# seshnadathur/victor

Measured on AMD Instinct MI355X. Metric: likelihood evals/sec (40 s-bins, 100 mu, l=0,2,4), higher is better.
Workload: dtype f64

## Files before the change

### victor_amd/csrc/vk_common.h

```cpp
#pragma once
#include <hip/hip_runtime.h>

#include "victor_hip.h"
#include "vk_devmath.h"
#include "vk_views.h"

namespace vk {

__device__ __forceinline__ int late_tid() {
  int t = threadIdx.x;
  asm volatile("" : "+v"(t));
  return t;
}


constexpr int kBlock = 256;
constexpr int kWaves = kBlock / 64;
constexpr int kMaxEll = 3;
constexpr int kVrVars = 5;
constexpr int kMaxParts = 8;


constexpr int kLikeRed = 4 * kWaves;
struct LikeArgs {
  const double* params;
  const double* theory;
  long long n;
  int N;
  int n_beta_d;
  const double* beta_d;
  const double* data;
  int n_beta_c;
  const double* beta_c;
  const double* prec;
  int grids_in_lds;
  const double* tri;
  const double* logdet;
  const double* eig;
  int like_form;
  double nmocks, nparams;
  double* lnl;
  double* chi2;
#ifdef VK_PHASES
  long long* stamps;
#endif
};

struct TheoryArgs {
  const double* params;
  long long n;
  int n_s, n_mu, n_x, n_ell;
  const double* s;
  const double* mu;
  const double* w_ell;
  const double* x;
  const double* w_x;
  const double* xw_scaled;
  double xw_max;
  const double* xgw;
  int n_xg;
  int n_beta_r;
  const double* beta_r;
  PPView xi, vr, sv;
  double iaH;
  double inv_sigma8;
  int rescale_from_ap;
  int matter_vt;
  double vt_amp;
  int sv_n_mu;
  double sv_mu_inv_h;
  const double* sv_mu;
  const double* sv2d;
  const double* sva;
  int sva_doubles;
  int uni_n;
  double uni_u0, uni_inv_h;
  const double* uni_sv_v;
  const double* uni_xi;
  const double* uni_xic;
  const double* uni_vb;
  const double* uni_v2;
  const double* uni_da;
  const double* uni_ge;
  const double* uni_dab;
  const double* uni_empb;
  int uni_lut_n;
  double uni_lut_inv_g;
  const unsigned short* uni_lut;
  const double* uni_knots;
  int matter_lb;
  int vr_beta_dep;
  const double* vr_emp;
  int from_data;
  int empirical;
  int rsd;
  int niter;
  int kaiser_approx;
  int coord_shift;
  int lanes_per_block;
  int sbins_per_item;
  int team;
  double* out;
  const double* exp_tab;
  const double* exp_tab_rep;
  const double* stage_mu;
  const double* image;
  double wsum[3];
  unsigned nx_magic;
  unsigned nmu_magic;
  unsigned ns_magic;
  int xi_out;
  int parts;
  int cells_per_item;
  int fuse;
  unsigned* counters;
  double* partial;
  int poll;
  int* poll_failed;
  LikeArgs like;
  double row0[VK_NPAR];
  int inline_row;
  int want_theory;
#ifdef VK_PHASES
  long long* stamps;
#endif
};

#ifdef VK_PHASES
#define VK_STAMP(a, k) do { if ((a).stamps && threadIdx.x == 0 && blockIdx.x < 4096) (a).stamps[blockIdx.x * 16 + (k)] = wall_clock64(); } while (0)
#else
#define VK_STAMP(a, k) do { } while (0)
#endif

struct PPLds {
  const double* knots;
  const double* coef;
  int n_int;
  int lead;
  double inv_h;
  double lo, hi, x_u0;
};

__device__ __forceinline__ int pp_interval(const PPLds& t, double u) {
  int i;
  if (t.inv_h != 0.0) {
    const int n_uniform = t.n_int - t.lead;
    const double tt = (u - t.x_u0) * fabs(t.inv_h);
    i = (int)tt;
    i = min(max(i, 0), n_uniform - 1) + t.lead;
    if (t.lead && u < t.x_u0) i = 0;
    if (t.inv_h < 0.0) {
      if (u < t.knots[i]) {
        i = max(i - 1, 0);
      } else if (u >= t.knots[i + 1]) {
        i = min(i + 1, t.n_int - 1);
      }
    }
  } else {
    int lo = 0, hi = t.n_int;
    while (hi - lo > 1) {
      int mid = (lo + hi) >> 1;
      if (u >= t.knots[mid]) lo = mid; else hi = mid;
    }
    i = lo;
  }
  return i;
}

__device__ __forceinline__ double pp_eval_at(const PPLds& t, int var, int i, double u) {
  const double dx = u - t.knots[i];
  const double* c = t.coef + ((size_t)var * t.n_int + i) * 4;
  return fma(fma(fma(c[3], dx, c[2]), dx, c[1]), dx, c[0]);
}

__device__ __forceinline__ double clampd(double u, double lo, double hi) { return fmin(fmax(u, lo), hi); }

__device__ __forceinline__ double wave_sum(double v) { return vkm::wave_sum(v); }

struct VelocityNode { double x, w; int last; };
__device__ __forceinline__ VelocityNode load_node(const double* xgw, int k) {
  typedef int node_words __attribute__((ext_vector_type(4)));
  typedef const node_words __attribute__((address_space(4))) * node_ptr;
  const node_words q = ((node_ptr)(unsigned long long)xgw)[k];
  VelocityNode n;
  n.x = __hiloint2double(q.y, q.x);
  n.w = __hiloint2double(q.w, q.z);
  n.last = q.w;
  return n;
}

template <int BYTES>
__device__ __forceinline__ void warm_kernarg_lines() {
  static_assert(BYTES <= 896, "extend the list of lines");
  const auto kp = __builtin_amdgcn_kernarg_segment_ptr();
  unsigned d0, d1, d2, d3, d4, d5, d6, d7, d8, d9, d10, d11;
  asm volatile(
      "s_load_dword %0, %12, 0x0\n\t"
      "s_load_dword %1, %12, 0x40\n\t"
      "s_load_dword %2, %12, 0x80\n\t"
      "s_load_dword %3, %12, 0xc0\n\t"
      "s_load_dword %4, %12, 0x100\n\t"
      "s_load_dword %5, %12, 0x140\n\t"
      "s_load_dword %6, %12, 0x180\n\t"
      "s_load_dword %7, %12, 0x1c0\n\t"
      "s_load_dword %8, %12, 0x200\n\t"
      "s_load_dword %9, %12, 0x240\n\t"
      "s_load_dword %10, %12, 0x280\n\t"
      "s_load_dword %11, %12, 0x2c0\n\t"
      "s_waitcnt lgkmcnt(0)"
      : "=&s"(d0), "=&s"(d1), "=&s"(d2), "=&s"(d3), "=&s"(d4), "=&s"(d5), "=&s"(d6), "=&s"(d7), "=&s"(d8), "=&s"(d9),
        "=&s"(d10), "=&s"(d11)
      : "s"(kp)
      : "memory");
  if constexpr (BYTES > 768) {
    unsigned e0, e1;
    if constexpr (BYTES > 832)
      asm volatile("s_load_dword %0, %2, 0x300\n\ts_load_dword %1, %2, 0x340\n\ts_waitcnt lgkmcnt(0)" : "=&s"(e0), "=&s"(e1) : "s"(kp) : "memory");
    else
      asm volatile("s_load_dword %0, %1, 0x300\n\ts_waitcnt lgkmcnt(0)" : "=&s"(e0) : "s"(kp) : "memory");
  }
}

__device__ __forceinline__ void store_shared(double* p, double v) {
  __hip_atomic_store(p, v, __ATOMIC_RELAXED, __HIP_MEMORY_SCOPE_AGENT);
}
__device__ __forceinline__ double load_shared(const double* p) {
  return __hip_atomic_load(p, __ATOMIC_RELAXED, __HIP_MEMORY_SCOPE_AGENT);
}

typedef double vk_shared2 __attribute__((ext_vector_type(2)));
__device__ __forceinline__ void load_shared_x8(const double* p, double (&v)[8]) {
  vk_shared2 a, b, c, d;
  asm volatile(
      "global_load_dwordx4 %0, %4, off sc1\n\t"
      "global_load_dwordx4 %1, %4, off offset:16 sc1\n\t"
      "global_load_dwordx4 %2, %4, off offset:32 sc1\n\t"
      "global_load_dwordx4 %3, %4, off offset:48 sc1\n\t"
      "s_waitcnt vmcnt(0)"
      : "=&v"(a), "=&v"(b), "=&v"(c), "=&v"(d)
      : "v"(p)
      : "memory");
  v[0] = a.x; v[1] = a.y; v[2] = b.x; v[3] = b.y; v[4] = c.x; v[5] = c.y; v[6] = d.x; v[7] = d.y;
}

constexpr unsigned long long kPollEmpty = 0x7ff8a5a57ff8a5a5ULL;
constexpr long long kPollTicks = 500000000LL;
__device__ __forceinline__ bool poll_is_empty(double v) { return (unsigned long long)__double_as_longlong(v) == kPollEmpty; }

__device__ __forceinline__ void drain_shared_stores() { asm volatile("s_waitcnt vmcnt(0)" ::: "memory"); }

__device__ __forceinline__ const double* param_row(const TheoryArgs& a, long long point) {
  return a.inline_row ? a.row0 : a.params + point * VK_NPAR;
}

__device__ __forceinline__ bool point_completed(unsigned* counters, long long point, unsigned total, int* flag) {
  drain_shared_stores();
  __syncthreads();
  if (threadIdx.x == 0) {
    const unsigned done = __hip_atomic_fetch_add(counters + point, 1u, __ATOMIC_RELAXED, __HIP_MEMORY_SCOPE_AGENT) + 1u;
    if (done == total) __hip_atomic_store(counters + point, 0u, __ATOMIC_RELAXED, __HIP_MEMORY_SCOPE_AGENT);
    *flag = done == total ? 1 : 0;
  }
  __syncthreads();
  return *flag != 0;
}

__device__ __forceinline__ double growth_amplitude(const TheoryArgs& a, const double* row, double fs8, double* av,
                                                   double* extra) {
  double growth = fs8 * a.inv_sigma8;
  double binv = 1.0;
  if (a.matter_lb) {
    const double bias = row[VK_P_BIAS];
    if (a.from_data) growth = row[VK_P_BETA] * bias;
    binv = vkm::recip(bias);
    *extra += bias;
  }
  if (a.matter_vt) growth = -3.0 * a.iaH * a.vt_amp * fs8;
  *av = 0.0;
  if (a.empirical && !a.matter_vt) {
    *av = row[VK_P_AV] * binv;
    *extra += *av;
  }
  return growth * binv;
}

struct PointScalars {
  double aperp, apar, inv_c, A, B;
  double G;
  double gD;
  double M, Q;
  double av;
  double inv_aperp, inv_apar;
  double poison;
};



__device__ __forceinline__ PointScalars point_scalars(const TheoryArgs& a, const double* row) {
  PointScalars ps;
  const double fs8 = row[VK_P_FSIGMA8];
  const double sigv = row[VK_P_SIGMAV];
  ps.aperp = row[VK_P_APERP];
  ps.apar = row[VK_P_APAR];
  const double eps = row[VK_P_EPSILON];
  double c;
  if (a.rescale_from_ap) {
    const int lane = threadIdx.x & 63;
    const double e2 = eps * eps - 1.0;
    const double h = (1.0 - 1e-10) / 49.0;
    double v = 0.0;
    if (lane < 50) {
      const double m = (lane == 49) ? 1.0 : fma((double)lane, h, 1e-10);
      double g, ir;
      vkm::sqrt_rsqrt(fma(1.0 - m * m, e2, 1.0), g, ir);
      v = ps.apar * g;
      if (lane == 0 || lane == 49) v *= 0.5;
    }
    c = wave_sum(v) * h;
  } else {
    c = row[VK_P_ASTAR];
  }
  ps.inv_c = vkm::recip(c);
  const double iaH_true = a.iaH * ps.apar;
  double extra = 0.0;
  const double gb = growth_amplitude(a, row, fs8, &ps.av, &extra);
  ps.B = sigv * iaH_true;
  ps.A = gb * vkm::recip(3.0 * iaH_true * sigv);
  ps.G = gb * (1.0 / 3.0);
  ps.gD = gb * ps.inv_c;
  ps.M = row[VK_P_M];
  ps.Q = row[VK_P_Q];
  ps.inv_aperp = vkm::recip(ps.aperp);
  ps.inv_apar = vkm::recip(ps.apar);
  ps.poison = 0.0 * (gb + sigv + ps.aperp + ps.apar + eps + c + ps.A + extra + (a.n_beta_r > 0 ? row[VK_P_BETA] : 0.0));
  return ps;
}

}
```

### victor_amd/csrc/vk_kernel_cells.h

```cpp
#pragma once
#include "vk_kernel_fast.h"

namespace vk {

struct CellsPlan {
  int mu, w, s, betar, da, v1, sva, image_end, acc, like, total;
};

__host__ __device__ inline int cells_range_bins(int n_mu, int cpi) { return (cpi + n_mu - 2) / n_mu + 1; }

__host__ __device__ inline CellsPlan make_cells_plan(int n_mu, int n_x, int n_s, int uni_n, int nlr, int n_beta_r,
                                                     int lut_n, int with_da, int cpi, int n_like, int n_sva = 0) {
  CellsPlan p;
  int o = fast_fixed_doubles(uni_n, nlr, lut_n);
  o = (o + 1) & ~1;
  p.mu = o;    o += 2 * n_mu;
  p.w = o;     o += kMaxEll * n_mu;
  p.s = o;     o += (n_s + 1) & ~1;
  p.betar = o; o += (n_beta_r + 1) & ~1;
  p.da = o;    o += with_da ? uni_n * 4 : 0;
  p.v1 = o;    o += with_da == 1 ? 0 : uni_n * 4;
  o = (o + 1) & ~1;
  p.sva = o;   o += (n_sva + 1) & ~1;
  p.image_end = o;
  int bins = cells_range_bins(n_mu, cpi);
  if (bins > n_s) bins = n_s;
  p.acc = o;   o += kMaxEll * (bins + 1) * kWaves;
  o = (o + 1) & ~1;
  p.like = o;  o += n_like > 0 ? like_lds_doubles(n_like) : 0;
  p.total = o;
  return p;
}

template <int NLR>
__device__ __forceinline__ void stage_cells(const TheoryArgs& a, const CellsPlan& pl, double* lds, int with_da) {
  const int tid = threadIdx.x;
  for (int i = tid; i < a.n_mu; i += kBlock) {
    const double m = a.mu[i];
    lds[pl.mu + 2 * i] = m;
    lds[pl.mu + 2 * i + 1] = sqrt(1.0 - m * m);
#pragma unroll
    for (int l = 0; l < kMaxEll; ++l) lds[pl.w + l * a.n_mu + i] = (l < a.n_ell) ? a.w_ell[l * a.n_mu + i] : 0.0;
  }
  for (int j = tid; j < a.n_s; j += kBlock) lds[pl.s + j] = a.s[j];
  stage_uni_records<NLR>(a, lds);
  if (with_da) stage_da<NLR>(a, lds + pl.da);
  if (with_da != 1) for (int e = tid; e < a.uni_n * 4; e += kBlock) lds[pl.v1 + e] = a.uni_sv_v[(e >> 2) * 8 + 4 + (e & 3)];
  if (a.n_beta_r > 0)
    for (int i = tid; i < a.n_beta_r; i += kBlock) lds[pl.betar + i] = a.beta_r[i];
  if (pl.image_end > pl.sva)
    for (int e = tid; e < a.sva_doubles; e += kBlock) lds[pl.sva + e] = a.sva[e];
}

template <int NL>
__device__ __forceinline__ void finish_point_ranges(const TheoryArgs& a, long long point, double beta, double poison, double* th,
                                                    bool gather, const double* lds_beta_r) {
  const int N = a.n_ell * a.n_s;
  const double w0 = a.wsum[0], w1 = a.wsum[1], w2 = a.wsum[2];
  const bool keep_out = !a.fuse || a.want_theory;
  LikePrefetch<kLikeRowsCells> pf;
  if (a.fuse) pf.issue(a.like, beta, late_tid(), lds_beta_r);
  for (int e = late_tid(); gather && e < N; e += kBlock) {
    const int l = (e >= 2 * a.n_s) ? 2 : (e >= a.n_s ? 1 : 0), j = e - l * a.n_s;
    const int q_first = (j * a.n_mu) / a.cells_per_item, q_last = (j * a.n_mu + a.n_mu - 1) / a.cells_per_item;
    double part[8];
    load_shared_x8(partial_slot(a, point, l, j), part);
    double v = 0.0;
#pragma unroll
    for (int c = 0; c < kMaxParts; ++c) v += (c <= q_last - q_first) ? part[c] : 0.0;
    v = v - (l == 0 ? w0 : (l == 1 ? w1 : w2)) + poison;
    if (keep_out) a.out[point * (long long)N + e] = v;
    th[e] = v;
  }
  __syncthreads();
  if (a.fuse) like_point_workgroup(a.like, point, beta, th, th + like_red_off(N), pf);
}

__device__ __forceinline__ double uniform_f64(double v) {
  return __hiloint2double(__builtin_amdgcn_readfirstlane(__double2hiint(v)), __builtin_amdgcn_readfirstlane(__double2loint(v)));
}

template <int NL>
__device__ __forceinline__ void project_trip(double g, bool first, bool second, const double* w_i, int n_mu, double* acc, int lstride, int lane) {
  const double ga = first ? g : 0.0, gb = second ? g : 0.0;
  double z[NL];
#pragma unroll
  for (int l = 0; l < NL; ++l) {
    const double w = w_i[l * n_mu];
    z[l] = vkm::fold32(w * ga, w * gb);
  }
  double x;
  int l_mine;
  bool mine;
  const int row = lane >> 4;
  if (NL == 3) {
    const double u = vkm::fold16(z[0], z[1]);
    const double v = vkm::fold16(z[2], 0.0);
    const bool up = (lane & 8) != 0;
    const double keep = up ? v : u, send = up ? u : v;
    x = keep + vkm::dpp_move<0x128, 0xF, true>(send);
    l_mine = up ? 2 : (row & 1);
    mine = (lane & 7) == 0 && !(up && (row & 1));
  } else {
    x = vkm::fold16(z[0], NL == 2 ? z[NL - 1] : 0.0);
    x += vkm::dpp_move<0x128, 0xF, true>(x);
    l_mine = row & 1;
    mine = (lane & 15) == 0 && (NL == 2 || !(row & 1));
  }
  x = vkm::octet_sum(x);
  if (mine) acc[l_mine * lstride + (lane >> 5) * kWaves] += x;
}

constexpr int kNodeBlock = 4;

template <int W, int NLR, int GRID, int FD, int CL, int SVA>
__device__ __forceinline__ void stream_block(const double* __restrict__ lds, const FastConsts& fc, const FastPoint& fp, double s_par,
                                             double sperp2, double sperp2x, const VelocityNode (&c)[kNodeBlock], double& g, double& gs) {
  UniHead h[W];
  double inv[W], p[W];
#pragma unroll
  for (int i = 0; i < W; ++i) {
    h[i] = uni_point_head<NLR, GRID, FD, 1, CL, 0, SVA>(lds, fc, 0.0, fma(-c[i].x, fp.Bk, s_par), sperp2, c[i].x, fp.fa, sperp2x);
    asm volatile("" : "+v"(h[i].SV), "+v"(h[i].ynum), "+v"(h[i].xi1));
    __builtin_amdgcn_sched_barrier(0);
  }
  if (W == 4) vkm::recip_shared4(h[0].SV, h[1 % W].SV, h[2 % W].SV, h[3 % W].SV, inv[0], inv[1 % W], inv[2 % W], inv[3 % W]);
  if (W == 3) vkm::recip_shared3(h[0].SV, h[1 % W].SV, h[2 % W].SV, inv[0], inv[1 % W], inv[2 % W]);
  if (W == 2) vkm::recip_shared2(h[0].SV, h[1 % W].SV, inv[0], inv[1 % W]);
  if (W == 1) inv[0] = vkm::recip_nr(h[0].SV);
#pragma unroll
  for (int i = 0; i < W; ++i) p[i] = uni_point_tail<0>(lds, h[i], inv[i], 0u);
#pragma unroll
  for (int i = 0; i < W; ++i) {
    gs = fma(inv[i], p[i], gs);
    if (c[i].last != 0) {
      asm volatile("" ::: "memory");
      g = fma(c[i].w, gs, g);
      gs = 0.0;
    }
  }
}

template <int NLR, int GRID, int FD, int CL, int SVA>
__device__ __forceinline__ double stream_cell(const TheoryArgs& a, const double* __restrict__ lds, const FastConsts& fc, const FastPoint& fp,
                                              double s_par, double sperp2, double sperp2x) {
  constexpr int W = kNodeBlock;
  double g = 0.0, gs = 0.0;
  const double* xgw = a.xgw;
  asm volatile("" : "+s"(xgw));
  VelocityNode nx[W];
#pragma unroll
  for (int i = 0; i < W; ++i) nx[i] = load_node(xgw, i);
  const int quads = a.n_xg / W;
  for (int b = 0; b < quads; ++b) {
    VelocityNode c[W];
#pragma unroll
    for (int i = 0; i < W; ++i) c[i] = nx[i];
#pragma unroll
    for (int i = 0; i < W; ++i) nx[i] = load_node(xgw, W * b + W + i);
    stream_block<W, NLR, GRID, FD, CL, SVA>(lds, fc, fp, s_par, sperp2, sperp2x, c, g, gs);
  }
  const int rest = a.n_xg - quads * W;
  if (rest == 3) stream_block<3, NLR, GRID, FD, CL, SVA>(lds, fc, fp, s_par, sperp2, sperp2x, nx, g, gs);
  else if (rest == 2) stream_block<2, NLR, GRID, FD, CL, SVA>(lds, fc, fp, s_par, sperp2, sperp2x, nx, g, gs);
  else if (rest == 1) stream_block<1, NLR, GRID, FD, CL, SVA>(lds, fc, fp, s_par, sperp2, sperp2x, nx, g, gs);
  return g;
}

template <int NLR, int NL, int GRID, int MODE, int SVA = 0>
__global__ __launch_bounds__(kBlock, (MODE == kModeStreaming && !SVA) || MODE == kModeKaiser ? 5 : 4) void vk_theory_cells_kernel(TheoryArgs a) {
  extern __shared__ double lds[];
  vkm::clamp_keeps_nan();
  warm_kernarg_lines<sizeof(TheoryArgs)>();
  const int N = a.n_ell * a.n_s;
  const int R = a.parts;
  const int cpi = a.cells_per_item;
  const bool xi_out = NL == 1 && a.xi_out != 0;
  const bool tail = !xi_out && (a.fuse || R > 1);
  CellsPlan pl = make_cells_plan(a.n_mu, a.n_x, a.n_s, a.uni_n, NLR, a.n_beta_r, a.uni_lut_n, mode_layout(MODE), xi_out ? 0 : cpi,
                                 tail ? N : 0, SVA ? a.sva_doubles : 0);
  pl.like = __builtin_amdgcn_readfirstlane(pl.like);
  const int tid = threadIdx.x;
  VK_STAMP(a, 0);
  if (a.image) copy_image(lds, a.image, pl.image_end);
  else stage_cells<NLR>(a, pl, lds, mode_layout(MODE));
  constexpr bool kHalf = MODE != kModeKaiser;
  const FastConsts fc = make_fast_consts<NLR>(a, kHalf, SVA ? pl.sva : 0);
  __syncthreads();
  VK_STAMP(a, 1);

  const int lane = tid & 63;
  const int wave = __builtin_amdgcn_readfirstlane(tid >> 6);
  const double* l_mu = lds + pl.mu;
  const double* l_w = lds + pl.w;
  const double* l_s = lds + pl.s;
  const int slots = xi_out ? 1 : min(cells_range_bins(a.n_mu, cpi), a.n_s) + 1;
  double* l_acc = lds + pl.acc;
  const unsigned items = (unsigned)a.n * (unsigned)R;
  const int all_cells = a.n_s * a.n_mu;

  {
    const unsigned item = blockIdx.x;
    if (item >= items) return;
    const long long point = item / (unsigned)R;
    const int q = (int)(item - (unsigned)point * (unsigned)R);
    const int c0 = q * cpi, c1 = min(c0 + cpi, all_cells);
    const int jf = (int)__umulhi((unsigned)c0, a.nmu_magic);
    const int nb = (int)__umulhi((unsigned)(c1 - 1), a.nmu_magic) - jf + 1;
    const double* row = a.params + point * VK_NPAR;
    constexpr bool kStream = !mode_has_da(MODE);
    PointScalars ps = point_scalars(a, row);
    if (kStream) ps.poison = uniform_f64(ps.poison);
    FastPoint fp = make_fast_point(ps, fc, kHalf);
    if (kStream) {
      fp.k_perp = uniform_f64(fp.k_perp);
      fp.k_par = uniform_f64(fp.k_par);
    }
    const double xi_max = kStream ? uniform_f64(a.xw_max * fabs(fp.Bk)) : 0.0;
    const double rlo2 = kStream ? uniform_f64(fc.rlo2) : 0.0, rhi2 = kStream ? uniform_f64(fc.rhi2) : 0.0;
    FastConsts fcs = fc;
    if (kStream && GRID == 0) {
      fcs.off = uniform_f64(fc.off);
      fcs.t_lo = uniform_f64(fc.t_lo);
      fcs.n_eps = uniform_f64(fc.n_eps);
    }
    constexpr int PV = MODE == kModeKaiser ? 0 : 1;
    __syncthreads();
    rebuild_point_tables<NLR, PV>(a, lds, pl.betar, pl.v1, row[VK_P_BETA], ps.av, mode_is_dispersion(MODE) ? -fp.Gk : fp.AVk,
                                  mode_has_da(MODE) ? lds + pl.da : nullptr);
    if (mode_has_da(MODE) && a.empirical && !a.vr_beta_dep) rebuild_da_emp(a, lds + pl.da, ps.av);
    for (int e = lane; e < kMaxEll * slots; e += 64) l_acc[e * kWaves + wave] = 0.0;
    __syncthreads();
    VK_STAMP(a, 2);
    for (int base = c0 + 64 * wave; base < c1; base += 64 * kWaves) {
      auto cell_of = [&](int e_, bool& live_, int& i_, int& j_) {
        live_ = e_ < c1;
        const unsigned ec = (unsigned)(live_ ? e_ : c1 - 1);
        const int hi = xi_out ? (a.n_s == 1 ? (int)ec : (int)__umulhi(ec, a.ns_magic)) : (int)__umulhi(ec, a.nmu_magic);
        const int lo = (int)ec - hi * (xi_out ? a.n_s : a.n_mu);
        j_ = xi_out ? lo : hi;
        i_ = xi_out ? hi : lo;
      };
      int i0, j;
      bool live0;
      cell_of(base + lane, live0, i0, j);
      const double sj = l_s[j];
      const vk_d2 mm = *reinterpret_cast<const vk_d2*>(l_mu + 2 * i0);
      const double s_perp = sj * fp.k_perp * mm.y;
      const double sperp2 = s_perp * s_perp;
      const double sperp2x = sperp2 * fp.fp2;
      const double s_par = sj * fp.k_par * mm.x;
      double g = 0.0;
      const bool inside = kStream && !__any(!cell_in_table(rlo2, rhi2, s_par, sperp2, xi_max));
      double gs = 0.0;
      if (MODE == kModeKaiser) {
        g = kaiser_value<NLR, GRID>(lds, lds + pl.da, fc, fp, ps.M, ps.Q, a.niter, a.coord_shift != 0, a.kaiser_approx != 0,
                                    a.rsd == VK_RSD_EUCLID, a.from_data != 0, s_par, sperp2);
      } else if (mode_is_dispersion(MODE)) {
        const double inv_den0 = disp_first_pass<NLR, GRID>(lds, fc, fp, a.niter, s_par, sperp2);
        for (int k = 0; k < a.n_xg; ++k) {
          const VelocityNode xw = load_node(a.xgw, k);
          gs += disp_value<NLR, GRID, MODE == kModeDispersionFromData, SVA>(lds, lds + pl.da, fc, fp, a.niter, fma(-xw.x, fp.Bk, s_par), inv_den0,
                                                                     sperp2, xw.x);
          if (xw.last != 0) {
            asm volatile("" ::: "memory");
            g = fma(xw.w, gs, g);
            gs = 0.0;
          }
        }
      } else if (inside) {
        g = stream_cell<NLR, GRID, MODE == kModeFromData, 0, SVA>(a, lds, fcs, fp, s_par, sperp2, sperp2x);
      } else {
        g = stream_cell<NLR, GRID, MODE == kModeFromData, GRID == 0 ? 2 : 1, SVA>(a, lds, fcs, fp, s_par, sperp2, sperp2x);
      }
      const int lane2 = kStream ? late_tid() & 63 : lane;
      const int e = base + lane2;
      int i = i0, j2 = j;
      bool live = live0;
      if (kStream) cell_of(e, live, i, j2);
      if (xi_out) {
        if (live) a.out[point * (long long)all_cells + e] = g - 1.0 + ps.poison;
        continue;
      }
      const int jj = j2 - jf;
      const int jj0 = __builtin_amdgcn_readfirstlane(jj);
      project_trip<NL>(g, live && jj == jj0, live && jj != jj0, l_w + i, a.n_mu, l_acc + jj0 * kWaves + wave, slots * kWaves, lane2);
    }
    if (xi_out) return;
    __syncthreads();
    double* th = lds + pl.like;
    for (int e = late_tid(); e < NL * nb; e += kBlock) {
      const int l = e / nb, jl = e - l * nb;
      const int j = jf + jl;
      const double* pa = l_acc + (l * slots + jl) * kWaves;
      const double sum = (pa[0] + pa[1]) + (pa[2] + pa[3]);
      if (R > 1) {
        store_shared(partial_slot(a, point, l, j) + (q - (j * a.n_mu) / cpi), sum);
      } else {
        const double v = sum - (l == 0 ? a.wsum[0] : (l == 1 ? a.wsum[1] : a.wsum[2])) + ps.poison;
        if (!a.fuse || a.want_theory) a.out[point * (long long)N + l * a.n_s + j] = v;
        if (tail) th[l * a.n_s + j] = v;
      }
    }
    VK_STAMP(a, 3);
    if (tail) {
      bool last = true;
      if (R > 1) {
        int* flag = reinterpret_cast<int*>(th + like_red_off(N) + kLikeRed + 2);
        last = point_completed(a.counters, point, (unsigned)R, flag);
      }
      VK_STAMP(a, 4);
      if (last) {
        finish_point_ranges<NL>(a, point, row[VK_P_BETA], ps.poison, th, R > 1, a.n_beta_r > 0 ? lds + pl.betar : nullptr);
        VK_STAMP(a, 5);
      }
      return;
    }
  }
}


}
```

Before: 2.849 million.

## Give each wave a contiguous cell run and accumulate per-bin partial sums in registers

In the streaming path, each wave now handles one contiguous chunk of cells instead of interleaving 64-cell trips across waves. Each lane keeps running per-multipole partial sums in registers and does a cross-lane reduction into LDS only when an s-bin boundary is crossed, replacing the per-trip project_trip reduction. The goal is fewer DPP reduction sequences and LDS accumulate operations per trip. In exchange it adds per-trip weight loads and boundary checks, and the per-wave work split can be uneven. A debug macro that records hardware wave IDs is also added behind VK_PHASES.

```diff
diff --git a/victor_amd/csrc/vk_common.h b/victor_amd/csrc/vk_common.h
--- a/victor_amd/csrc/vk_common.h
+++ b/victor_amd/csrc/vk_common.h
@@ -128,8 +128,11 @@
 
 #ifdef VK_PHASES
 #define VK_STAMP(a, k) do { if ((a).stamps && threadIdx.x == 0 && blockIdx.x < 4096) (a).stamps[blockIdx.x * 16 + (k)] = wall_clock64(); } while (0)
+#define VK_STAMP_HWID(a) do { if ((a).stamps && (threadIdx.x & 63) == 0 && blockIdx.x < 4096) \
+    reinterpret_cast<unsigned short*>((a).stamps + blockIdx.x * 16 + 7)[threadIdx.x >> 6] = (unsigned short)__builtin_amdgcn_s_getreg((15 << 11) | 4); } while (0)
 #else
 #define VK_STAMP(a, k) do { } while (0)
+#define VK_STAMP_HWID(a) do { } while (0)
 #endif
 
 struct PPLds {
diff --git a/victor_amd/csrc/vk_kernel_cells.h b/victor_amd/csrc/vk_kernel_cells.h
--- a/victor_amd/csrc/vk_kernel_cells.h
+++ b/victor_amd/csrc/vk_kernel_cells.h
@@ -111,6 +111,18 @@
   if (mine) acc[l_mine * lstride + (lane >> 5) * kWaves] += x;
 }
 
+template <int NL>
+__device__ __forceinline__ void project_bin(const double (&z)[NL], double* acc, int lstride, int lane) {
+  const double lo = vkm::fold32(z[0], NL > 1 ? z[NL > 1 ? 1 : 0] : 0.0);
+  double x = vkm::fold16(lo, NL == 3 ? vkm::fold32(z[NL - 1], 0.0) : 0.0);
+  x += vkm::dpp_move<0x128, 0xF, true>(x);
+  x = vkm::octet_sum(x);
+  const int row = lane >> 4;
+  const int l_mine = row == 0 ? 0 : (row == 2 ? 1 : 2);
+  const bool mine = (lane & 15) == 0 && (row == 0 || (row == 2 && NL > 1) || (row == 1 && NL == 3));
+  if (mine) acc[l_mine * lstride] += x;
+}
+
 constexpr int kNodeBlock = 4;
 
 template <int W, int NLR, int GRID, int FD, int CL, int SVA>
@@ -232,7 +244,25 @@
     for (int e = lane; e < kMaxEll * slots; e += 64) l_acc[e * kWaves + wave] = 0.0;
     __syncthreads();
     VK_STAMP(a, 2);
-    for (int base = c0 + 64 * wave; base < c1; base += 64 * kWaves) {
+    VK_STAMP_HWID(a);
+    const bool runs = kStream && !xi_out;
+    int b0 = 0, bend = 0, jlow = 0, bin_end = 0;
+    double psum[NL];
+    if (kStream) {
+      b0 = c0 + 64 * wave;
+      bend = c1;
+#pragma unroll
+      for (int l = 0; l < NL; ++l) psum[l] = 0.0;
+      if (runs) {
+        const int trips = (c1 - c0 + 63) >> 6;
+        b0 = c0 + 64 * ((trips * wave) >> 2);
+        bend = min(c0 + 64 * ((trips * (wave + 1)) >> 2), c1);
+        const int jb = (int)__umulhi((unsigned)b0, a.nmu_magic);
+        jlow = jb - jf;
+        bin_end = (jb + 1) * a.n_mu;
+      }
+    }
+    for (int base = kStream ? b0 : c0 + 64 * wave; base < (kStream ? bend : c1); base += kStream && runs ? 64 : 64 * kWaves) {
       auto cell_of = [&](int e_, bool& live_, int& i_, int& j_) {
         live_ = e_ < c1;
         const unsigned ec = (unsigned)(live_ ? e_ : c1 - 1);
@@ -283,10 +313,34 @@
         continue;
       }
       const int jj = j2 - jf;
+      if (kStream) {
+        const double* w_i = l_w + i;
+        double wl[NL];
+#pragma unroll
+        for (int l = 0; l < NL; ++l) wl[l] = w_i[l * a.n_mu];
+        if (live && jj == jlow) {
+          asm volatile("" ::: "memory");
+#pragma unroll
+          for (int l = 0; l < NL; ++l) psum[l] = fma(wl[l], g, psum[l]);
+        }
+        if (base + 64 >= bin_end) {
+          project_bin<NL>(psum, l_acc + jlow * kWaves + wave, slots * kWaves, lane2);
+          ++jlow;
+          bin_end += a.n_mu;
+          const bool next = live && jj == jlow;
+#pragma unroll
+          for (int l = 0; l < NL; ++l) psum[l] = next ? wl[l] * g : 0.0;
+        }
+        continue;
+      }
       const int jj0 = __builtin_amdgcn_readfirstlane(jj);
       project_trip<NL>(g, live && jj == jj0, live && jj != jj0, l_w + i, a.n_mu, l_acc + jj0 * kWaves + wave, slots * kWaves, lane2);
     }
     if (xi_out) return;
+    if (kStream && b0 < bend) {
+      const int jend = (int)__umulhi((unsigned)(bend - 1), a.nmu_magic) - jf;
+      if (jlow <= jend) project_bin<NL>(psum, l_acc + jlow * kWaves + wave, slots * kWaves, late_tid() & 63);
+    }
     __syncthreads();
     double* th = lds + pl.like;
     for (int e = late_tid(); e < NL * nb; e += kBlock) {
```

Result: no change. 2.858 million, median of 6 (+0.3%).
